# fverdoja/Fast-3D-Pointcloud-Segmentation

Measured on AMD Instinct MI355X. Metric: Mpoints/sec segmented end-to-end, 1M-pt RGB-D frames, higher is better.
Workload: dtype f32

## Files before the change

### __graft_entry__.py

```python
import importlib
import os
import subprocess
import sys

ROOT = os.path.dirname(os.path.abspath(__file__))
PKG = "fast-3d-pointcloud-segmentation_amd"


def _run(cmd):
    print("+", " ".join(cmd), flush=True)
    subprocess.run(cmd, check=True)


def build() -> None:
    _run(["make", "-C", os.path.join(ROOT, PKG, "csrc")])
    _run(["make", "-C", os.path.join(ROOT, "oracle")])
    _run(["make", "-C", os.path.join(ROOT, "tests", "emul")])
    _run(["make", "-C", os.path.join(ROOT, "tests", "devprobe")])
    _run(["make", "-C", os.path.join(ROOT, "tests", "kernprobe")])
    if ROOT not in sys.path:
        sys.path.insert(0, ROOT)
    P = importlib.import_module(PKG)
    lib = P.load_library()
    assert lib.f3ds_version() >= 120
    P.check_library_is_current(lib)


def smoke() -> None:
    import ctypes
    import numpy as np
    if ROOT not in sys.path:
        sys.path.insert(0, ROOT)
    sys.path.insert(0, os.path.join(ROOT, "tests"))
    P = importlib.import_module(PKG)
    from conftest import CpuChecker
    if P.device_count() < 1:
        raise RuntimeError("smoke(): no HIP device visible; libf3ds has no CPU fallback")
    pts = P.synth_frame(0, 7, 160, 120, 30)
    prm = P.launch_params(voxel_res=0.02, seed_res=0.2)
    ctx = P.Context(0)
    labels = ctx.segment(pts, prm)
    ora = CpuChecker(os.path.join(ROOT, "oracle", "libf3ds_oracle.so"), "f3ds_oracle")
    rc, olabels, ores, oh = ora.segment(pts, prm)
    assert rc == 0
    assert np.array_equal(labels, olabels), "HIP labels differ from the oracle"
    assert ctx.result.n_regions == ores.n_regions and ctx.result.n_merges == ores.n_merges
    print("smoke ok: N=%d V=%d S=%d E=%d merges=%d regions=%d  (%.2f ms on device 0)" % (
        len(pts), ctx.result.n_voxels, ctx.result.n_supervoxels, ctx.result.n_edges, ctx.result.n_merges, ctx.result.n_regions, ctx.result.ms_total))
    ctx.close()


if __name__ == "__main__":
# ... 4 lines not shown
```

### fast-3d-pointcloud-segmentation_amd/csrc/f3ds_hip.hip

```cpp
#include <hip/hip_runtime.h>

#include <algorithm>
#include <cmath>
#include <atomic>
#include <map>
#include <chrono>
#include <cstdio>
#include <cstdlib>
#include <cstring>
#include <string>
#include <type_traits>
#include <mutex>
#include <set>
#include <vector>

#include "../../include/f3ds.h"
#include "f3ds_algo.h"
#include "f3ds_glasbey.h"
#include "f3ds_eval.h"
#include "f3ds_dev.h"
#include "f3ds_levels.h"
#include "f3ds_eval_levels.h"

using namespace f3ds;
// ... 425 lines not shown
    rec<d_scan_single>(c, 1u, 0u, tiles, nt);
    rec<d_seg_write>(c, nt, 0u, c->ks, n, invalid, ks, tiles, seg_start, &c->d_dc->n_voxels, &c->d_dc->n_valid);
    return F3DS_OK;
}
int seg_vox_tiles(f3ds_ctx* c, int code_bits, int tile_bits) {
    const uint32_t n = c->n;
    const uint32_t ntiles = (n + VT_TILE - 1u) / VT_TILE;
    const uint64_t dcap64 = (uint64_t)ntiles * VT_ENT_MAX;
    if (code_bits + tile_bits + VT_CNT_BITS > 64 || dcap64 > 0x7fffffffull || (uint64_t)ntiles * VT_TAB > 0x7fffffffull) return F3DS_ERR_UNSUPPORTED;
    const uint32_t dcap = (uint32_t)dcap64;
    const uint64_t fin = c->h_dc->n_finite;
    const uint32_t capV = (uint32_t)std::max<uint64_t>(256u, std::min<uint64_t>(fin, dcap));
    c->vox_cap = capV;
    uint64_t *k0, *k1; uint32_t *ploc, *v0, *v1, *part, *vkey, *vcount, *seg_start, *list; uint2* bo_te; float* vf; int* pt_voxel;
    const uint32_t nchunks = (dcap + DS_CHUNK - 1u) / DS_CHUNK;
    ENSURE(c->pslot, n, ploc); ENSURE(c->keys0, dcap, k0); ENSURE(c->keys1, dcap, k1); ENSURE(c->vals0, dcap, v0); ENSURE(c->vals1, dcap, v1);
    { uint32_t* w; ENSURE(c->hcnt, (size_t)ntiles * VT_TAB * 2 + 2u * nchunks, w); bo_te = reinterpret_cast<uint2*>(w); part = w + (size_t)ntiles * VT_TAB * 2; }
    ENSURE(c->vkey, (size_t)capV * 3, vkey); ENSURE(c->vcount, capV, vcount); ENSURE(c->vf, (size_t)capV * 12, vf);
    ENSURE(c->seg_start, (size_t)capV + 1, seg_start); ENSURE(c->vlist, n, list); ENSURE(c->pt_voxel, n, pt_voxel);
    { uint32_t *f, *incl; ENSURE(c->flags, capV, f); ENSURE(c->incl, capV, incl); }
    c->idxbits = -1; c->ks = nullptr; c->vs = nullptr;
    rec<d_tile_keys>(c, std::min<uint32_t>(ntiles, (uint32_t)g_grid_cap * 16u), 0u, c->d_pts, n, c->fa, c->d_grid, ploc, k0, v0, dcap, tile_bits, c->d_dc);
    uint64_t* ks; uint32_t* vs;
    int rc = radix_sort(c, k0, v0, k1, v1, dcap, code_bits + tile_bits, &ks, &vs, VT_CNT_BITS, &c->d_dc->seg_count);
    if (rc) return rc;
    rec<d_desc_part>(c, nchunks, 0u, ks, dcap, tile_bits, part, c->d_dc);
    rec<d_desc_offsets>(c, 1u, 0u, part, dcap, capV, seg_start, c->d_dc);
    rec<d_desc_apply>(c, nchunks, 0u, ks, vs, dcap, capV, tile_bits, c->fa, c->d_grid, part, bo_te, seg_start, vkey, c->d_dc);
    rec<d_tile_place>(c, std::min<uint32_t>(ntiles, (uint32_t)g_grid_cap * 16u), 0u, ploc, n, bo_te, list, pt_voxel, c->d_dc);
    rec<d_voxel_list_accum>(c, std::min<uint32_t>(grid_wide(capV, 256), std::max<uint32_t>(64u, grid_wide(n / 8u, 256))), 0u, c->d_pts, list, seg_start, c->fa, vf, vcount, c->d_dc, capV);
    c->vox_hashed = true;
    return F3DS_OK;
}
int seg_voxels(f3ds_ctx* c) {
    const uint32_t V = c->V, n = c->n;
    uint32_t *vkey, *vcount, *hvals; float *vf; int *nbr, *nbrT; uint64_t* hkeys;
    if (c->vox_hashed) {
        const uint32_t hc2 = pow2_ge((size_t)V * 2 + 16);
        c->hmask = hc2 - 1;
        ENSURE(c->nbr, (size_t)V * 27, nbr); ENSURE(c->nbrT, (size_t)V * 27, nbrT); ENSURE(c->hkeys, hc2, hkeys); ENSURE(c->hvals, hc2, hvals);
        rec_fill(c, hkeys, 0xFFFFFFFFu, (size_t)hc2 * 8);
        rec<d_vox_hash>(c, 1u, 0u, c->vkey.p, V, c->d_grid, hkeys, hvals, c->hmask);
        rec<d_neighbors>(c, grid_wide((size_t)V * 27, 256), 0u, c->vkey.p, c->d_dc, c->d_grid, hkeys, hvals, c->hmask, nbr, nbrT);
        return F3DS_OK;
    }
    const uint32_t hcap = pow2_ge((size_t)V * 2 + 16);
    c->hmask = hcap - 1;
    ENSURE(c->vkey, (size_t)V * 3, vkey); ENSURE(c->vcount, V, vcount); ENSURE(c->vf, (size_t)V * 12, vf);
    ENSURE(c->nbr, (size_t)V * 27, nbr); ENSURE(c->nbrT, (size_t)V * 27, nbrT); ENSURE(c->hkeys, hcap, hkeys); ENSURE(c->hvals, hcap, hvals);
    rec_fill(c, hkeys, 0xFFFFFFFFu, (size_t)hcap * 8);
    if (g_sw.split_voxel_accum) {
        P16* spts; ENSURE(c->spts, n, spts);
        rec<d_point_gather>(c, grid_wide(n, 256), 0u, c->d_pts, c->vs, c->ks, c->idxbits < 0 ? 0 : c->idxbits, c->incl.p, n, c->d_dc, spts, c->pt_voxel.p);
        rec<d_voxel_accum>(c, grid_wide(V, 256), 0u, spts, c->ks, c->idxbits < 0 ? 0 : c->idxbits, c->seg_start.p, c->d_dc, c->fa, c->d_grid, vkey, vcount, vf, hkeys, hvals, c->hmask);
    } else
        rec<d_voxel_gather_accum>(c, grid_wide(V, 256), 0u, c->d_pts, c->vs, c->ks, c->idxbits < 0 ? 0 : c->idxbits, c->seg_start.p, n, c->d_dc, c->fa, c->d_grid, vkey, vcount, vf, hkeys, hvals, c->hmask, c->pt_voxel.p);
    rec<d_neighbors>(c, grid_wide((size_t)V * 27, 256), 0u, vkey, c->d_dc, c->d_grid, hkeys, hvals, c->hmask, nbr, nbrT);
    return F3DS_OK;
}
int seg_normals(f3ds_ctx* c) {
    const uint32_t nt = (c->V + NT_TILE - 1) / NT_TILE;
    uint32_t *tn1, *tord, *tslots;
    ENSURE(c->tile_n1, nt, tn1); ENSURE(c->tile_ord, (size_t)nt * NT_RING1, tord); ENSURE(c->tile_slots, (size_t)nt * SW_SLOT_WORDS * NT_TILE, tslots);
#ifdef F3DS_NORMALS_LOOP
    static const uint32_t budget = dev_getenv("F3DS_NORMALS_WGS") ? (uint32_t)atoi(dev_getenv("F3DS_NORMALS_WGS")) : 0u;
#else
    static const uint32_t budget = 0u;
#endif
    const uint32_t share = budget ? std::max(2u, budget / (uint32_t)g_batch_frames) : nt;
    const int nthr_env = g_sw.normals_threads;
    const uint32_t holes = g_sw.tile_holes;
    if (nthr_env ? nthr_env == 256 : g_batch_frames >= 16)
        rec<d_normals_t<256>>(c, std::min(nt, share), 0u, c->vf.p, c->nbr.p, c->d_dc, tn1, tord, tslots, holes);
    else
        rec<d_normals_t<384>>(c, std::min(nt, share), 0u, c->vf.p, c->nbr.p, c->d_dc, tn1, tord, tslots, holes);
    return F3DS_OK;
}
int seg_seed_grid(f3ds_ctx* c) {
    const uint32_t V = c->V;
    float* boxes; const float* vf = c->vf.p;
    const uint32_t nchunks = (V + SEED_CHUNK - 1) / SEED_CHUNK;
    ENSURE(c->boxes, (size_t)nchunks * 6, boxes);
    rec<d_chunkbox>(c, nchunks, 0u, vf, c->d_dc, boxes);
    rec<d_seed_grow>(c, 1u, 0u, vf, boxes, c->d_dc, c->prm.seed_res, c->d_sgrid);
    return F3DS_OK;
}
int seg_seed_cells(f3ds_ctx* c, int sort_bits, int max_sdepth) {
    const uint32_t V = c->V;
    uint32_t *ckey, *cell_start, *v0, *v1; uint64_t *k0 = c->keys0.p, *k1 = c->keys1.p;
    ENSURE(c->vals0, V, v0); ENSURE(c->vals1, V, v1);
    ENSURE(c->ckey, (size_t)V * 3, ckey); ENSURE(c->cell_start, (size_t)V + 1, cell_start);
// ... 1484 lines not shown
```

### fast-3d-pointcloud-segmentation_amd/csrc/f3ds_kernels.inc

```


namespace {

struct P16 { float x, y, z; uint32_t rgba; };

struct DevCounters {
    unsigned long long n_finite;
    uint32_t bbox[6];
    uint32_t bbox_any;
    uint32_t n_valid;
    uint32_t n_voxels;
    uint32_t n_cells;
    uint32_t n_seeds;
    uint32_t n_edges;
    uint32_t n_alive;
    uint32_t n_merges;
    uint32_t n_regions;
    uint32_t n_events;
    int error;
    int r_overflow;
    float lambda;
    uint32_t seg_count;
    uint32_t n_ghosts;
    int depth;
// ... 245 lines not shown
        __syncthreads();
    #pragma unroll
        for (int s = 0; s < RS_STRIPS; ++s) {
            uint32_t i = wbase + s * 64 + lane_id();
            const bool valid = i < n;
            const uint32_t d = (uint32_t)(k[s] >> shift) & mask;
            uint64_t peers = __ballot(valid);
            for (int b = 0; b < bits; ++b) {
                uint64_t m = __ballot(valid && ((d >> b) & 1u));
                peers &= ((d >> b) & 1u) ? m : ~m;
            }
            uint32_t pos = 0;
            if (valid) pos = wcount[w][d] + (uint32_t)__popcll(peers & lanemask_lt());
            __builtin_amdgcn_wave_barrier();
            if (valid && (peers & lanemask_lt()) == 0ull) wcount[w][d] += (uint32_t)__popcll(peers);
            __builtin_amdgcn_wave_barrier();
            if (valid) keys_out[pos] = k[s];
        }
    }
};

struct FrameArgs {
    int use_transform, fold_negative_z, leaf_order;
    float voxel_res, seed_res, w_color, w_spatial, w_normal;
};

__device__ inline P16 load_point(const P16* pts, size_t i) {
    const uint4 q = reinterpret_cast<const uint4*>(pts)[i];
    P16 p;
    p.x = __uint_as_float(q.x); p.y = __uint_as_float(q.y); p.z = __uint_as_float(q.z); p.rgba = q.w;
    return p;
}

__device__ inline bool vt_compact(int depth) { return depth <= 10; }
__device__ inline uint32_t vt_key30(unsigned x, unsigned y, unsigned z) { return (x << 20) | (y << 10) | z; }
template <bool WG_SCOPE>
__device__ inline void vt_insert(uint64_t* hkeys, uint32_t* hvals, uint32_t hmask, int depth, unsigned x, unsigned y, unsigned z, uint32_t v) {
    const bool compact = vt_compact(depth);
    const unsigned long long pk = compact ? (((unsigned long long)vt_key30(x, y, z) << 32) | v) : (unsigned long long)n_pack_key(x, y, z);
    uint32_t h = (uint32_t)hash64(compact ? (uint64_t)vt_key30(x, y, z) : (uint64_t)pk) & hmask;
    for (;;) {
        unsigned long long expect = HASH_EMPTY;
        const bool won = WG_SCOPE ? __hip_atomic_compare_exchange_strong((unsigned long long*)&hkeys[h], &expect, pk, __ATOMIC_RELAXED, __ATOMIC_RELAXED, __HIP_MEMORY_SCOPE_WORKGROUP)
                                  : __hip_atomic_compare_exchange_strong((unsigned long long*)&hkeys[h], &expect, pk, __ATOMIC_RELAXED, __ATOMIC_RELAXED, __HIP_MEMORY_SCOPE_AGENT);
        if (won || (!compact && expect == pk)) { if (!compact) hvals[h] = v; return; }
        h = (h + 1u) & hmask;
    }
}
__device__ inline int vt_find(const uint64_t* hkeys, const uint32_t* hvals, uint32_t hmask, bool compact, unsigned x, unsigned y, unsigned z) {
    if (compact) {
        const uint32_t ck = vt_key30(x, y, z);
        uint32_t h = (uint32_t)hash64((uint64_t)ck) & hmask;
        for (;;) {
            const uint64_t e = hkeys[h];
            if ((uint32_t)(e >> 32) == ck) return (int)(uint32_t)e;
            if (e == HASH_EMPTY) return -1;
            h = (h + 1u) & hmask;
        }
    }
    const uint64_t pk = n_pack_key(x, y, z);
    uint32_t h = (uint32_t)hash64(pk) & hmask;
    for (;;) {
        const uint64_t k = hkeys[h];
        if (k == pk) return (int)hvals[h];
        if (k == HASH_EMPTY) return -1;
        h = (h + 1u) & hmask;
    }
}
struct d_bbox {
    static constexpr int BLOCK = 256;
    __device__ void operator()(const P16* pts, uint32_t n, FrameArgs fa, DevCounters* dc) const {
        float mn[3] = {F3DS_FLT_MAX, F3DS_FLT_MAX, F3DS_FLT_MAX}, mx[3] = {-F3DS_FLT_MAX, -F3DS_FLT_MAX, -F3DS_FLT_MAX};
        uint32_t nfin = 0, any = 0;
        for (uint32_t i = BIX * blockDim.x + threadIdx.x; i < n; i += gridDim.x * blockDim.x) {
            P16 p = load_point(pts, i);
            float x = p.x, y = p.y, z = p.z;
            n_prelude(z, fa.fold_negative_z);
            if (n_finite3(x, y, z)) nfin++;
            n_transform(x, y, z, fa.use_transform);
            if (!n_finite3(x, y, z)) continue;
            any = 1;
            if (x < mn[0]) mn[0] = x;
            if (y < mn[1]) mn[1] = y;
            if (z < mn[2]) mn[2] = z;
            if (x > mx[0]) mx[0] = x;
            if (y > mx[1]) mx[1] = y;
            if (z > mx[2]) mx[2] = z;
        }
    #pragma unroll
        for (int d = 32; d >= 1; d >>= 1) {
            for (int a = 0; a < 3; ++a) {
                float t = __shfl_xor(mn[a], d, 64); if (t < mn[a]) mn[a] = t;
                t = __shfl_xor(mx[a], d, 64); if (t > mx[a]) mx[a] = t;
            }
            nfin += __shfl_xor(nfin, d, 64);
            any |= __shfl_xor(any, d, 64);
        }
        __shared__ float smn[4][3], smx[4][3];
        __shared__ uint32_t sfin[4], sany[4];
// ... 100 lines not shown
    __device__ void operator()(const uint64_t* keys, uint32_t n, uint64_t limit, int shift, const uint32_t* tile_offsets, uint32_t* seg_start, uint32_t* nseg_out, uint32_t* nvalid_out) const {
        if (BIX > 0 && BIX * SCAN_TILE >= n) return;
        const uint32_t base = BIX * SCAN_TILE + threadIdx.x * SCAN_ITEMS;
        uint64_t k[SCAN_ITEMS + 1]; uint32_t mask, tot;
        const uint32_t cnt = seg_heads_of_thread(keys, n, limit, shift, base, k, &mask);
        uint32_t run = tile_offsets[BIX] + block_incl_scan<SCAN_THREADS>(cnt, &tot) - cnt;
#pragma unroll
        for (int i = 0; i < SCAN_ITEMS; ++i) {
            const uint32_t pos = base + (uint32_t)i;
            if (mask & (1u << i)) seg_start[run++] = pos;
            if (pos < n && k[i] < limit && (pos + 1u == n || k[i + 1] >= limit)) { seg_start[run] = pos + 1u; *nseg_out = run; *nvalid_out = pos + 1u; }
        }
    }
};
struct d_point_gather {
    static constexpr int BLOCK = 256;
    __device__ void operator()(const P16* pts, const uint32_t* vals, const uint64_t* keys, int idxbits, const uint32_t* incl, uint32_t n, const DevCounters* dc, P16* spts,
                               int* pt_voxel) const {
        const uint32_t nv = dc->n_valid;
        for (uint32_t i = BIX * blockDim.x + threadIdx.x; i < n; i += gridDim.x * blockDim.x) {
            const uint32_t idx = vals ? vals[i] : (uint32_t)(keys[i] & ((1ull << idxbits) - 1ull));
            if (i < nv) {
                const P16 p = load_point(pts, idx);
                *reinterpret_cast<float4*>(spts + i) = make_float4(p.x, p.y, p.z, __uint_as_float(p.rgba));
                pt_voxel[idx] = (int)(incl[i] - 1u);
            } else pt_voxel[idx] = -1;
        }
    }
};
struct d_voxel_accum {
    static constexpr int BLOCK = 256;
    __device__ void operator()(const P16* spts, const uint64_t* keys, int keyshift, const uint32_t* seg_start,
                                                    const DevCounters* dc, FrameArgs fa, const GridInfo* gp, uint32_t* vkey, uint32_t* vcount,
                                                    float* vf, uint64_t* hkeys, uint32_t* hvals, uint32_t hmask) const {
        const uint32_t V = dc->n_voxels;
        const int depth = gp->depth;
        for (uint32_t v = BIX * blockDim.x + threadIdx.x; v < V; v += gridDim.x * blockDim.x) {
            const uint32_t s = seg_start[v], e = seg_start[v + 1];
            float sx = 0, sy = 0, sz = 0, sr = 0, sg = 0, sb = 0;
            for (uint32_t i = s; i < e; ++i) {
                P16 p = load_point(spts, i);
                float z = p.z; n_prelude(z, fa.fold_negative_z);
                sx += p.x; sy += p.y; sz += z;
                sr += (float)((p.rgba >> 16) & 255u); sg += (float)((p.rgba >> 8) & 255u); sb += (float)(p.rgba & 255u);
            }
            const uint32_t cnt = e - s;
            const float c = (float)cnt;
            float4* row = reinterpret_cast<float4*>(vf + (size_t)v * 12);
            row[0] = make_float4(sx / c, sy / c, sz / c, sr / c);
            row[1] = make_float4(sg / c, sb / c, 0.0f, 0.0f);
            row[2] = make_float4(0.0f, 0.0f, 0.0f, 0.0f);
            vcount[v] = cnt;
            uint64_t code = keys[s] >> keyshift;
            if (fa.leaf_order == 1) code = (~code) & ((1ull << (3 * depth)) - 1ull);
            unsigned k[3];
            n_demorton(code, depth, k);
            vkey[v * 3] = k[0]; vkey[v * 3 + 1] = k[1]; vkey[v * 3 + 2] = k[2];
            vt_insert<false>(hkeys, hvals, hmask, depth, k[0], k[1], k[2], v);
        }
    }
};
constexpr uint32_t VG_CHUNK = 1024;
struct d_voxel_gather_accum {
    static constexpr int BLOCK = 256;
    __device__ void operator()(const P16* pts, const uint32_t* vals, const uint64_t* keys, int keyshift, const uint32_t* seg_start, uint32_t n,
                               const DevCounters* dc, FrameArgs fa, const GridInfo* gp, uint32_t* vkey, uint32_t* vcount,
                               float* vf, uint64_t* hkeys, uint32_t* hvals, uint32_t hmask, int* pt_voxel) const {
        __shared__ __attribute__((aligned(16))) uint4 buf[VG_CHUNK];
        __shared__ uint32_t ibuf[VG_CHUNK], vbuf[VG_CHUNK];
        const uint32_t V = dc->n_voxels, nv = dc->n_valid;
        const int depth = gp->depth;
        const uint64_t imask = (1ull << keyshift) - 1ull;
        const uint32_t tid = threadIdx.x;
        for (uint32_t i = nv + BIX * blockDim.x + tid; i < n; i += gridDim.x * blockDim.x) pt_voxel[vals ? vals[i] : (uint32_t)(keys[i] & imask)] = -1;
        for (uint32_t vb = BIX * 256u; vb < V; vb += gridDim.x * 256u) {
            const uint32_t v = vb + tid;
            const bool mine = v < V;
            const uint32_t s = mine ? seg_start[v] : 0u, e = mine ? seg_start[v + 1] : 0u;
            const uint32_t p0 = seg_start[vb], p1 = seg_start[vb + 256u < V ? vb + 256u : V];
            float sx = 0, sy = 0, sz = 0, sr = 0, sg = 0, sb = 0;
            for (uint32_t c0 = p0; c0 < p1; c0 += VG_CHUNK) {
                const uint32_t c1 = p1 - c0 < VG_CHUNK ? p1 : c0 + VG_CHUNK;
                uint32_t idx[VG_CHUNK / 256];
        #pragma unroll
                for (uint32_t j = 0; j < VG_CHUNK / 256; ++j) { const uint32_t i = c0 + j * 256u + tid; const uint32_t ii = i < c1 ? i : c1 - 1u; idx[j] = vals ? vals[ii] : (uint32_t)(keys[ii] & imask); }
                uint4 q[VG_CHUNK / 256];
        #pragma unroll
                for (uint32_t j = 0; j < VG_CHUNK / 256; ++j) q[j] = reinterpret_cast<const uint4*>(pts)[idx[j]];
        #pragma unroll
                for (uint32_t j = 0; j < VG_CHUNK / 256; ++j) { buf[j * 256u + tid] = q[j]; ibuf[j * 256u + tid] = idx[j]; }
                __syncthreads();
                const uint32_t a = s > c0 ? s : c0, b = e < c1 ? e : c1;
                for (uint32_t i = a; i < b; ++i) {
                    const uint4 w = buf[i - c0];
                    float z = __uint_as_float(w.z); n_prelude(z, fa.fold_negative_z);
                    sx += __uint_as_float(w.x); sy += __uint_as_float(w.y); sz += z;
                    sr += (float)((w.w >> 16) & 255u); sg += (float)((w.w >> 8) & 255u); sb += (float)(w.w & 255u);
                    vbuf[i - c0] = v;
                }
                __syncthreads();
        #pragma unroll
                for (uint32_t j = 0; j < VG_CHUNK / 256; ++j) { const uint32_t pp = j * 256u + tid; if (c0 + pp < c1) pt_voxel[ibuf[pp]] = (int)vbuf[pp]; }
                __syncthreads();
            }
            if (!mine) continue;
            const uint32_t cnt = e - s;
            const float c = (float)cnt;
            float4* row = reinterpret_cast<float4*>(vf + (size_t)v * 12);
            row[0] = make_float4(sx / c, sy / c, sz / c, sr / c);
            row[1] = make_float4(sg / c, sb / c, 0.0f, 0.0f);
            row[2] = make_float4(0.0f, 0.0f, 0.0f, 0.0f);
            vcount[v] = cnt;
            uint64_t code = keys[s] >> keyshift;
            if (fa.leaf_order == 1) code = (~code) & ((1ull << (3 * depth)) - 1ull);
            unsigned k[3];
            n_demorton(code, depth, k);
            vkey[v * 3] = k[0]; vkey[v * 3 + 1] = k[1]; vkey[v * 3 + 2] = k[2];
            vt_insert<false>(hkeys, hvals, hmask, depth, k[0], k[1], k[2], v);
        }
    }
};

#ifndef F3DS_VT_TILE
#define F3DS_VT_TILE 4096
#endif
constexpr uint32_t VT_TILE = F3DS_VT_TILE;
constexpr uint32_t VT_TAB = VT_TILE / 2;
constexpr int VT_CNT_BITS = 14;
static_assert(VT_TILE < (1u << VT_CNT_BITS), "a tile's point count must fit the count field");
constexpr uint32_t VT_ENT_MAX = VT_TAB * 5 / 8;
constexpr uint32_t VL_MAX_RUN = 256;
constexpr uint32_t VOX_NONE = 0xFFFFFFFFu;
__device__ inline void run_of_lane(bool valid, uint32_t w0, uint32_t w1, bool* head, int* head_lane, uint32_t* run_len) {
    const int lane = lane_id();
    const uint32_t p0 = __shfl_up(w0, 1, 64), p1 = __shfl_up(w1, 1, 64);
    const bool pv = __shfl_up((int)valid, 1, 64) != 0;
    const bool h = valid && (lane == 0 || !pv || p0 != w0 || p1 != w1);
    const uint64_t hm = __ballot(h), vm = __ballot(valid);
    const uint64_t le = lane == 63 ? ~0ull : ((2ull << lane) - 1ull);
    const int hl = valid ? 63 - __builtin_clzll(hm & le) : lane;
    const uint64_t above = hl == 63 ? 0ull : ~((2ull << hl) - 1ull);
    const uint64_t stop = (hm | ~vm) & above;
    *head = h; *head_lane = hl; *run_len = (uint32_t)((stop ? __builtin_ctzll(stop) : 64) - hl);
}
struct d_tile_keys {
    static constexpr int BLOCK = 256;
    __device__ void operator()(const P16* pts, uint32_t n, FrameArgs fa, const GridInfo* gp, uint32_t* ploc, uint64_t* dkeys, uint32_t* dvals,
                               uint32_t dcap, int tile_bits, DevCounters* dc) const {
        __shared__ unsigned long long tkey[VT_TAB];
        __shared__ uint32_t tcnt[VT_TAB];
        __shared__ uint32_t tbits[2][VT_TAB / 32];
// ... 198 lines not shown
    static constexpr int BLOCK = 256;
    __device__ void operator()(const uint32_t* ploc, uint32_t n, const uint2* bo_te, uint32_t* list, int* pt_voxel, const DevCounters* dc) const {
        __shared__ uint2 tab[VT_TAB];
        if (dc->ev_overflow) return;
        const uint32_t ntiles = (n + VT_TILE - 1u) / VT_TILE;
        for (uint32_t tile = BIX; tile < ntiles; tile += gridDim.x) {
            const uint32_t t0 = tile * VT_TILE, t1 = n - t0 < VT_TILE ? n : t0 + VT_TILE;
            constexpr uint32_t PF = 4;
            uint32_t pl[PF];
    #pragma unroll
            for (uint32_t j = 0; j < PF; ++j) { const uint32_t i = t0 + j * 256u + threadIdx.x; pl[j] = i < t1 ? ploc[i] : VOX_NONE; }
            __syncthreads();
            for (uint32_t e = threadIdx.x; e < VT_TAB; e += 256u) tab[e] = bo_te[(size_t)tile * VT_TAB + e];
            __syncthreads();
            for (uint32_t i0 = t0; i0 < t1; i0 += 256u * PF) {
                uint32_t nx[PF];
    #pragma unroll
                for (uint32_t j = 0; j < PF; ++j) { const uint32_t i = i0 + (PF + j) * 256u + threadIdx.x; nx[j] = i < t1 ? ploc[i] : VOX_NONE; }
    #pragma unroll
                for (uint32_t j = 0; j < PF; ++j) {
                    const uint32_t i = i0 + j * 256u + threadIdx.x;
                    if (i >= t1) continue;
                    if (pl[j] == VOX_NONE) { pt_voxel[i] = -1; continue; }
                    const uint2 bo = tab[pl[j] >> 16];
                    list[bo.x + (pl[j] & 0xFFFFu)] = i;
                    pt_voxel[i] = (int)bo.y;
                }
    #pragma unroll
                for (uint32_t j = 0; j < PF; ++j) pl[j] = nx[j];
            }
        }
    }
};
struct d_vox_hash {
    static constexpr bool LATENCY_KERNEL = true;
    static constexpr int BLOCK = 1024;
    __device__ void operator()(const uint32_t* vkey, uint32_t V, const GridInfo* gp, uint64_t* hkeys, uint32_t* hvals, uint32_t hmask) const {
        if (BIX) return;
        const int depth = gp->depth;
        constexpr uint32_t PF = 4;
        for (uint32_t v0 = threadIdx.x; v0 < V; v0 += blockDim.x * PF) {
            unsigned k[PF][3];
    #pragma unroll
            for (uint32_t j = 0; j < PF; ++j) { const uint32_t v = v0 + j * blockDim.x, vv = v < V ? v : 0u; k[j][0] = vkey[vv * 3]; k[j][1] = vkey[vv * 3 + 1]; k[j][2] = vkey[vv * 3 + 2]; }
    #pragma unroll
            for (uint32_t j = 0; j < PF; ++j) { const uint32_t v = v0 + j * blockDim.x; if (v < V) vt_insert<true>(hkeys, hvals, hmask, depth, k[j][0], k[j][1], k[j][2], v); }
        }
    }
};
struct d_voxel_list_accum {
    static constexpr int BLOCK = 256;
    __device__ void operator()(const P16* pts, uint32_t* list, const uint32_t* seg_start, FrameArgs fa, float* vf, uint32_t* vcount, DevCounters* dc, uint32_t capV) const {
        __shared__ __attribute__((aligned(16))) uint4 buf[VG_CHUNK];
        if (dc->ev_overflow) return;
        const uint32_t V = dc->n_voxels < capV ? dc->n_voxels : capV;
        const bool disorder = dc->vox_disorder != 0u;
        const uint32_t tid = threadIdx.x;
        for (uint32_t vb = BIX * 256u; vb < V; vb += gridDim.x * 256u) {
            const uint32_t v = vb + tid;
            const bool mine = v < V;
            const uint32_t s = mine ? seg_start[v] : 0u, e = mine ? seg_start[v + 1] : 0u;
            const uint32_t p0 = seg_start[vb], p1 = seg_start[vb + 256u < V ? vb + 256u : V];
            if (__syncthreads_or(e - s > VL_MAX_RUN)) { if (tid == 0) { dc->error = F3DS_ERR_UNSUPPORTED; dc->ev_overflow = 6; } return; }
            if (disorder) {
                for (uint32_t a = s + 1u; a < e; ++a) {
                    const uint32_t x = list[a];
                    uint32_t b = a;
                    while (b > s && list[b - 1u] > x) { list[b] = list[b - 1u]; --b; }
                    if (b != a) list[b] = x;
                }
                __threadfence_block();
                __syncthreads();
            }
            float sx = 0, sy = 0, sz = 0, sr = 0, sg = 0, sb = 0;
            for (uint32_t c0 = p0; c0 < p1; c0 += VG_CHUNK) {
                const uint32_t c1 = p1 - c0 < VG_CHUNK ? p1 : c0 + VG_CHUNK;
                uint32_t idx[VG_CHUNK / 256];
        #pragma unroll
                for (uint32_t j = 0; j < VG_CHUNK / 256; ++j) { const uint32_t i = c0 + j * 256u + tid; idx[j] = list[i < c1 ? i : c1 - 1u]; }
// ... 4 lines not shown
                for (uint32_t j = 0; j < VG_CHUNK / 256; ++j) buf[j * 256u + tid] = q[j];
                __syncthreads();
                const uint32_t a = s > c0 ? s : c0, b = e < c1 ? e : c1;
                for (uint32_t i = a; i < b; ++i) {
                    const uint4 w = buf[i - c0];
                    float z = __uint_as_float(w.z); n_prelude(z, fa.fold_negative_z);
                    sx += __uint_as_float(w.x); sy += __uint_as_float(w.y); sz += z;
                    sr += (float)((w.w >> 16) & 255u); sg += (float)((w.w >> 8) & 255u); sb += (float)(w.w & 255u);
                }
                __syncthreads();
            }
            if (!mine) continue;
            const float c = (float)(e - s);
            vcount[v] = e - s;
            float4* row = reinterpret_cast<float4*>(vf + (size_t)v * 12);
            row[0] = make_float4(sx / c, sy / c, sz / c, sr / c);
            row[1] = make_float4(sg / c, sb / c, 0.0f, 0.0f);
            row[2] = make_float4(0.0f, 0.0f, 0.0f, 0.0f);
        }
    }
};
__device__ inline int hash_find(const uint64_t* hkeys, const uint32_t* hvals, uint32_t hmask, uint64_t pk) {
    uint32_t h = (uint32_t)hash64(pk) & hmask;
    for (;;) {
        uint64_t k = hkeys[h];
        if (k == pk) return (int)hvals[h];
        if (k == HASH_EMPTY) return -1;
        h = (h + 1u) & hmask;
    }
}

struct d_neighbors {
    static constexpr int BLOCK = 256;
    __device__ void operator()(const uint32_t* vkey, const DevCounters* dc, const GridInfo* gp, const uint64_t* hkeys,
                                                  const uint32_t* hvals, uint32_t hmask, int* nbr, int* nbrT) const {
        __shared__ int tr[27][65];
        const uint32_t V = dc->n_voxels;
        const unsigned max_key = gp->max_key;
        const bool compact = vt_compact(gp->depth);
        for (uint32_t vb = BIX * 64u; vb < V; vb += gridDim.x * 64u) {
            const uint32_t nv = V - vb < 64u ? V - vb : 64u, np = nv * 27u;
            for (uint32_t tl = threadIdx.x; tl < np; tl += 256u) {
                const uint32_t vl = tl / 27u, s = tl - vl * 27u, v = vb + vl;
                const int d[3] = {(int)(s / 9u) - 1, (int)((s / 3u) % 3u) - 1, (int)(s % 3u) - 1};
                bool ok = true; unsigned k[3];
                for (int a = 0; a < 3; ++a) {
                    long long q = (long long)vkey[v * 3 + a] + d[a];
                    if (q < 0 || q > (long long)max_key) ok = false;
                    k[a] = (unsigned)q;
                }
                const int u = ok ? vt_find(hkeys, hvals, hmask, compact, k[0], k[1], k[2]) : -1;
                nbr[(size_t)vb * 27u + tl] = u;
                tr[s][vl] = u;
            }
            __syncthreads();
            for (uint32_t r = threadIdx.x; r < 27u * 64u; r += 256u) {
                const uint32_t s = r >> 6, vl = r & 63u;
                if (vl < nv) nbrT[(size_t)s * V + vb + vl] = tr[s][vl];
            }
            __syncthreads();
        }
    }
};
constexpr int NT_TILE = 128;
constexpr int NT_HCAP = 2048;
#ifndef F3DS_NT_SLOTS
#define F3DS_NT_SLOTS 896
#endif
#ifndef F3DS_NT_RING1
#define F3DS_NT_RING1 448
#endif
constexpr int NT_SLOTS = F3DS_NT_SLOTS;
constexpr int NT_RING1 = F3DS_NT_RING1;
constexpr uint16_t NT_NONE = 0xFFFFu;
constexpr uint32_t NT_HNONE = 0x3FFu;
constexpr uint32_t NT_ORD_LIMIT = (1u << 22) - 2u;
static_assert(NT_SLOTS < 1023, "slot numbers share a word with the ordinal");
constexpr uint16_t NT_ZERO = NT_SLOTS;
constexpr uint32_t SW_TILE_NONE = 0xFFFFFFFFu;
constexpr int SW_SLOT_BITS = 9;
constexpr int SW_SLOT_WORDS = (27 * SW_SLOT_BITS + 31) / 32;
static_assert(NT_RING1 < (1 << SW_SLOT_BITS), "a list position must fit its bit field");
__device__ __forceinline__ void sw_slots_pack(const uint32_t pos[27], uint32_t w[SW_SLOT_WORDS]) {
#pragma unroll
// ... 3034 lines not shown
```

### fast-3d-pointcloud-segmentation_amd/csrc/f3ds_numerics.h

```cpp
#ifndef F3DS_NUMERICS_H_
#define F3DS_NUMERICS_H_

#include "f3ds_math.h"

namespace f3ds {

#define F3DS_FLT_MAX 3.402823466e+38f
#define F3DS_FLT_MIN 1.175494351e-38f
#define F3DS_FLT_EPS 1.192092896e-07f

F3DS_HD float n_sqrtf(float x) { return __builtin_sqrtf(x); }
F3DS_HD double n_sqrt(double x) { return __builtin_sqrt(x); }
F3DS_HD bool n_finite3(float x, float y, float z) { return m_isfinitef(x) && m_isfinitef(y) && m_isfinitef(z); }
F3DS_HD float n_nanf() { return m_from_bitsf(0x7fc00000u); }

struct GridInfo {
    double min[3];
    double max[3];
    double res;
    int depth;
    unsigned max_key;
    int error;
    int empty;
};
// ... 55 lines not shown
    v = (v | (v << 8)) & 0x0300F00Fu;
    v = (v | (v << 4)) & 0x030C30C3u;
    v = (v | (v << 2)) & 0x09249249u;
    return v;
}
F3DS_HD uint64_t n_spread3_21(uint64_t v) {
    v = (v | (v << 32)) & 0x001F00000000FFFFull;
    v = (v | (v << 16)) & 0x001F0000FF0000FFull;
    v = (v | (v << 8)) & 0x100F00F00F00F00Full;
    v = (v | (v << 4)) & 0x10C30C30C30C30C3ull;
    v = (v | (v << 2)) & 0x1249249249249249ull;
    return v;
}
F3DS_HD uint64_t n_morton(unsigned x, unsigned y, unsigned z, int depth) {
    if (depth <= 10) {
        const uint32_t m = (1u << depth) - 1u;
        return (uint64_t)((n_spread3_10(x & m) << 2) | (n_spread3_10(y & m) << 1) | n_spread3_10(z & m));
    }
    const uint64_t m = (1ull << depth) - 1ull;
    return (n_spread3_21(x & m) << 2) | (n_spread3_21(y & m) << 1) | n_spread3_21(z & m);
}
F3DS_HD void n_demorton(uint64_t c, int depth, unsigned key[3]) {
    unsigned x = 0, y = 0, z = 0;
    for (int b = depth - 1; b >= 0; --b) {
        unsigned d = (unsigned)(c >> (3 * b)) & 7u;
        x = (x << 1) | ((d >> 2) & 1u);
        y = (y << 1) | ((d >> 1) & 1u);
        z = (z << 1) | (d & 1u);
    }
    key[0] = x; key[1] = y; key[2] = z;
}
F3DS_HD uint64_t n_pack_key(unsigned x, unsigned y, unsigned z) {
    return ((uint64_t)x << 42) | ((uint64_t)y << 21) | (uint64_t)z;
}

F3DS_HD void n_roots2(float b, float c, float r[3]) {
    r[0] = 0.0f;
    float d = (float)((double)(b * b) - 4.0 * (double)c);
    if (d < 0.0f) d = 0.0f;
    float sd = n_sqrtf(d);
    r[2] = 0.5f * (b + sd);
    r[1] = 0.5f * (b - sd);
}
template <class K = m_lit> F3DS_HD void n_roots(float m00, float m01, float m02, float m11, float m12, float m22, float r[3], K mc = K()) {
    float c0 = m00 * m11 * m22 + 2.0f * m01 * m02 * m12 - m00 * m12 * m12 - m11 * m02 * m02 - m22 * m01 * m01;
    float c1 = m00 * m11 - m01 * m01 + m00 * m22 - m02 * m02 + m11 * m22 - m12 * m12;
    float c2 = m00 + m11 + m22;
    if (m_absf(c0) < F3DS_FLT_EPS) { n_roots2(c2, c1, r); return; }
    const float inv3 = (float)(1.0 / 3.0);
    const float sqrt3 = 1.7320508075688772f;
    float c2_3 = c2 * inv3;
    float a_3 = (c1 - c2 * c2_3) * inv3;
    if (a_3 > 0.0f) a_3 = 0.0f;
    float half_b = 0.5f * (c0 + c2_3 * (2.0f * c2_3 * c2_3 - c1));
    float q = half_b * half_b + a_3 * a_3 * a_3;
    if (q > 0.0f) q = 0.0f;
    float rho = n_sqrtf(-a_3);
    float theta = m_atan2f(n_sqrtf(-q), half_b, mc) * inv3;
    float ct = m_cosf(theta, mc), st = m_sinf(theta, mc);
    r[0] = c2_3 + 2.0f * rho * ct;
    r[1] = c2_3 - rho * (ct + sqrt3 * st);
    r[2] = c2_3 - rho * (ct - sqrt3 * st);
    float t;
    if (r[0] >= r[1]) { t = r[0]; r[0] = r[1]; r[1] = t; }
    if (r[1] >= r[2]) {
        t = r[1]; r[1] = r[2]; r[2] = t;
// ... 188 lines not shown
```

Baseline: 3638.

## Replace per-voxel hash table with 4x4x4 block occupancy table for neighbor lookup

```diff
diff --git a/__graft_entry__.py b/__graft_entry__.py
--- a/__graft_entry__.py
+++ b/__graft_entry__.py
@@ -18,6 +18,7 @@
     _run(["make", "-C", os.path.join(ROOT, "tests", "emul")])
     _run(["make", "-C", os.path.join(ROOT, "tests", "devprobe")])
     _run(["make", "-C", os.path.join(ROOT, "tests", "kernprobe")])
+    _run(["make", "-C", os.path.join(ROOT, "tests", "blockprobe")])
     if ROOT not in sys.path:
         sys.path.insert(0, ROOT)
     P = importlib.import_module(PKG)
diff --git a/fast-3d-pointcloud-segmentation_amd/csrc/f3ds_hip.hip b/fast-3d-pointcloud-segmentation_amd/csrc/f3ds_hip.hip
--- a/fast-3d-pointcloud-segmentation_amd/csrc/f3ds_hip.hip
+++ b/fast-3d-pointcloud-segmentation_amd/csrc/f3ds_hip.hip
@@ -481,31 +481,32 @@
     c->vox_hashed = true;
     return F3DS_OK;
 }
+int seg_neighbors(f3ds_ctx* c, uint32_t wgs) {
+    const uint32_t V = c->V;
+    const bool blocks = c->h_dc->depth <= N_BLOCK_DEPTH_MAX;
+    const uint32_t cap = blocks ? pow2_ge((size_t)V + 16) : pow2_ge((size_t)V * 2 + 16);
+    const size_t words = blocks ? (size_t)cap * 2 : cap;
+    uint32_t* hvals = nullptr; int *nbr, *nbrT; uint64_t* hkeys;
+    c->hmask = cap - 1;
+    ENSURE(c->nbr, (size_t)V * 27, nbr); ENSURE(c->nbrT, (size_t)V * 27, nbrT); ENSURE(c->hkeys, words, hkeys);
+    if (!blocks) ENSURE(c->hvals, cap, hvals);
+    rec_fill(c, hkeys, 0xFFFFFFFFu, words * 8);
+    rec<d_vox_table>(c, wgs, 0u, c->vkey.p, V, c->d_grid, hkeys, hvals, c->hmask);
+    rec<d_neighbors>(c, grid_wide((size_t)V * 27, 256), 0u, c->vkey.p, c->d_dc, c->d_grid, c->fa.leaf_order, hkeys, hvals, c->hmask, nbr, nbrT);
+    return F3DS_OK;
+}
 int seg_voxels(f3ds_ctx* c) {
     const uint32_t V = c->V, n = c->n;
-    uint32_t *vkey, *vcount, *hvals; float *vf; int *nbr, *nbrT; uint64_t* hkeys;
-    if (c->vox_hashed) {
-        const uint32_t hc2 = pow2_ge((size_t)V * 2 + 16);
-        c->hmask = hc2 - 1;
-        ENSURE(c->nbr, (size_t)V * 27, nbr); ENSURE(c->nbrT, (size_t)V * 27, nbrT); ENSURE(c->hkeys, hc2, hkeys); ENSURE(c->hvals, hc2, hvals);
-        rec_fill(c, hkeys, 0xFFFFFFFFu, (size_t)hc2 * 8);
-        rec<d_vox_hash>(c, 1u, 0u, c->vkey.p, V, c->d_grid, hkeys, hvals, c->hmask);
-        rec<d_neighbors>(c, grid_wide((size_t)V * 27, 256), 0u, c->vkey.p, c->d_dc, c->d_grid, hkeys, hvals, c->hmask, nbr, nbrT);
-        return F3DS_OK;
-    }
-    const uint32_t hcap = pow2_ge((size_t)V * 2 + 16);
-    c->hmask = hcap - 1;
+    if (c->vox_hashed) return seg_neighbors(c, 1u);
+    uint32_t *vkey, *vcount; float *vf;
     ENSURE(c->vkey, (size_t)V * 3, vkey); ENSURE(c->vcount, V, vcount); ENSURE(c->vf, (size_t)V * 12, vf);
-    ENSURE(c->nbr, (size_t)V * 27, nbr); ENSURE(c->nbrT, (size_t)V * 27, nbrT); ENSURE(c->hkeys, hcap, hkeys); ENSURE(c->hvals, hcap, hvals);
-    rec_fill(c, hkeys, 0xFFFFFFFFu, (size_t)hcap * 8);
     if (g_sw.split_voxel_accum) {
         P16* spts; ENSURE(c->spts, n, spts);
         rec<d_point_gather>(c, grid_wide(n, 256), 0u, c->d_pts, c->vs, c->ks, c->idxbits < 0 ? 0 : c->idxbits, c->incl.p, n, c->d_dc, spts, c->pt_voxel.p);
-        rec<d_voxel_accum>(c, grid_wide(V, 256), 0u, spts, c->ks, c->idxbits < 0 ? 0 : c->idxbits, c->seg_start.p, c->d_dc, c->fa, c->d_grid, vkey, vcount, vf, hkeys, hvals, c->hmask);
+        rec<d_voxel_accum>(c, grid_wide(V, 256), 0u, spts, c->ks, c->idxbits < 0 ? 0 : c->idxbits, c->seg_start.p, c->d_dc, c->fa, c->d_grid, vkey, vcount, vf);
     } else
-        rec<d_voxel_gather_accum>(c, grid_wide(V, 256), 0u, c->d_pts, c->vs, c->ks, c->idxbits < 0 ? 0 : c->idxbits, c->seg_start.p, n, c->d_dc, c->fa, c->d_grid, vkey, vcount, vf, hkeys, hvals, c->hmask, c->pt_voxel.p);
-    rec<d_neighbors>(c, grid_wide((size_t)V * 27, 256), 0u, vkey, c->d_dc, c->d_grid, hkeys, hvals, c->hmask, nbr, nbrT);
-    return F3DS_OK;
+        rec<d_voxel_gather_accum>(c, grid_wide(V, 256), 0u, c->d_pts, c->vs, c->ks, c->idxbits < 0 ? 0 : c->idxbits, c->seg_start.p, n, c->d_dc, c->fa, c->d_grid, vkey, vcount, vf, c->pt_voxel.p);
+    return seg_neighbors(c, grid_for(V, 4096));
 }
 int seg_normals(f3ds_ctx* c) {
     const uint32_t nt = (c->V + NT_TILE - 1) / NT_TILE;
diff --git a/fast-3d-pointcloud-segmentation_amd/csrc/f3ds_kernels.inc b/fast-3d-pointcloud-segmentation_amd/csrc/f3ds_kernels.inc
--- a/fast-3d-pointcloud-segmentation_amd/csrc/f3ds_kernels.inc
+++ b/fast-3d-pointcloud-segmentation_amd/csrc/f3ds_kernels.inc
@@ -301,32 +301,24 @@
     return p;
 }
 
-__device__ inline bool vt_compact(int depth) { return depth <= 10; }
-__device__ inline uint32_t vt_key30(unsigned x, unsigned y, unsigned z) { return (x << 20) | (y << 10) | z; }
-template <bool WG_SCOPE>
-__device__ inline void vt_insert(uint64_t* hkeys, uint32_t* hvals, uint32_t hmask, int depth, unsigned x, unsigned y, unsigned z, uint32_t v) {
-    const bool compact = vt_compact(depth);
-    const unsigned long long pk = compact ? (((unsigned long long)vt_key30(x, y, z) << 32) | v) : (unsigned long long)n_pack_key(x, y, z);
-    uint32_t h = (uint32_t)hash64(compact ? (uint64_t)vt_key30(x, y, z) : (uint64_t)pk) & hmask;
+__device__ inline bool vt_blocks(int depth) { return depth <= N_BLOCK_DEPTH_MAX; }
+constexpr uint32_t BT_EMPTY = 0xFFFFFFFFu;
+struct __attribute__((aligned(16))) BtEntry { uint32_t key, base; unsigned long long vacant; };
+static_assert(sizeof(BtEntry) == 16, "one 16-byte load per probe");
+template <class T> __device__ inline bool vt_cas(T* p, T* expect, T v, bool agent) {
+    return agent ? __hip_atomic_compare_exchange_strong(p, expect, v, __ATOMIC_RELAXED, __ATOMIC_RELAXED, __HIP_MEMORY_SCOPE_AGENT)
+                 : __hip_atomic_compare_exchange_strong(p, expect, v, __ATOMIC_RELAXED, __ATOMIC_RELAXED, __HIP_MEMORY_SCOPE_WORKGROUP);
+}
+__device__ inline void vt_insert(uint64_t* hkeys, uint32_t* hvals, uint32_t hmask, bool agent, unsigned x, unsigned y, unsigned z, uint32_t v) {
+    const unsigned long long pk = (unsigned long long)n_pack_key(x, y, z);
+    uint32_t h = (uint32_t)hash64((uint64_t)pk) & hmask;
     for (;;) {
         unsigned long long expect = HASH_EMPTY;
-        const bool won = WG_SCOPE ? __hip_atomic_compare_exchange_strong((unsigned long long*)&hkeys[h], &expect, pk, __ATOMIC_RELAXED, __ATOMIC_RELAXED, __HIP_MEMORY_SCOPE_WORKGROUP)
-                                  : __hip_atomic_compare_exchange_strong((unsigned long long*)&hkeys[h], &expect, pk, __ATOMIC_RELAXED, __ATOMIC_RELAXED, __HIP_MEMORY_SCOPE_AGENT);
-        if (won || (!compact && expect == pk)) { if (!compact) hvals[h] = v; return; }
+        if (vt_cas((unsigned long long*)&hkeys[h], &expect, pk, agent) || expect == pk) { hvals[h] = v; return; }
         h = (h + 1u) & hmask;
     }
 }
-__device__ inline int vt_find(const uint64_t* hkeys, const uint32_t* hvals, uint32_t hmask, bool compact, unsigned x, unsigned y, unsigned z) {
-    if (compact) {
-        const uint32_t ck = vt_key30(x, y, z);
-        uint32_t h = (uint32_t)hash64((uint64_t)ck) & hmask;
-        for (;;) {
-            const uint64_t e = hkeys[h];
-            if ((uint32_t)(e >> 32) == ck) return (int)(uint32_t)e;
-            if (e == HASH_EMPTY) return -1;
-            h = (h + 1u) & hmask;
-        }
-    }
+__device__ inline int vt_find(const uint64_t* hkeys, const uint32_t* hvals, uint32_t hmask, unsigned x, unsigned y, unsigned z) {
     const uint64_t pk = n_pack_key(x, y, z);
     uint32_t h = (uint32_t)hash64(pk) & hmask;
     for (;;) {
@@ -334,6 +326,24 @@
         if (k == pk) return (int)hvals[h];
         if (k == HASH_EMPTY) return -1;
         h = (h + 1u) & hmask;
+    }
+}
+__device__ inline BtEntry* bt_entry(BtEntry* tab, uint32_t tmask, bool agent, uint32_t bk) {
+    uint32_t h = (uint32_t)hash64((uint64_t)bk) & tmask;
+    for (;;) {
+        uint32_t expect = BT_EMPTY;
+        if (vt_cas(&tab[h].key, &expect, bk, agent) || expect == bk) return &tab[h];
+        h = (h + 1u) & tmask;
+    }
+}
+__device__ inline int bt_find(const BtEntry* tab, uint32_t tmask, int leaf_order, unsigned x, unsigned y, unsigned z) {
+    const uint32_t bk = n_block_key(x, y, z);
+    uint32_t h = (uint32_t)hash64((uint64_t)bk) & tmask;
+    for (;;) {
+        const uint4 e = reinterpret_cast<const uint4*>(tab)[h];
+        if (e.x == bk) return n_block_ordinal(e.y, ~(((uint64_t)e.w << 32) | (uint64_t)e.z), n_block_cell(x, y, z), leaf_order);
+        if (e.x == BT_EMPTY) return -1;
+        h = (h + 1u) & tmask;
     }
 }
 struct d_bbox {
@@ -500,7 +510,7 @@
     static constexpr int BLOCK = 256;
     __device__ void operator()(const P16* spts, const uint64_t* keys, int keyshift, const uint32_t* seg_start,
                                                     const DevCounters* dc, FrameArgs fa, const GridInfo* gp, uint32_t* vkey, uint32_t* vcount,
-                                                    float* vf, uint64_t* hkeys, uint32_t* hvals, uint32_t hmask) const {
+                                                    float* vf) const {
         const uint32_t V = dc->n_voxels;
         const int depth = gp->depth;
         for (uint32_t v = BIX * blockDim.x + threadIdx.x; v < V; v += gridDim.x * blockDim.x) {
@@ -524,7 +534,6 @@
             unsigned k[3];
             n_demorton(code, depth, k);
             vkey[v * 3] = k[0]; vkey[v * 3 + 1] = k[1]; vkey[v * 3 + 2] = k[2];
-            vt_insert<false>(hkeys, hvals, hmask, depth, k[0], k[1], k[2], v);
         }
     }
 };
@@ -533,7 +542,7 @@
     static constexpr int BLOCK = 256;
     __device__ void operator()(const P16* pts, const uint32_t* vals, const uint64_t* keys, int keyshift, const uint32_t* seg_start, uint32_t n,
                                const DevCounters* dc, FrameArgs fa, const GridInfo* gp, uint32_t* vkey, uint32_t* vcount,
-                               float* vf, uint64_t* hkeys, uint32_t* hvals, uint32_t hmask, int* pt_voxel) const {
+                               float* vf, int* pt_voxel) const {
         __shared__ __attribute__((aligned(16))) uint4 buf[VG_CHUNK];
         __shared__ uint32_t ibuf[VG_CHUNK], vbuf[VG_CHUNK];
         const uint32_t V = dc->n_voxels, nv = dc->n_valid;
@@ -584,7 +593,6 @@
             unsigned k[3];
             n_demorton(code, depth, k);
             vkey[v * 3] = k[0]; vkey[v * 3 + 1] = k[1]; vkey[v * 3 + 2] = k[2];
-            vt_insert<false>(hkeys, hvals, hmask, depth, k[0], k[1], k[2], v);
         }
     }
 };
@@ -849,19 +857,51 @@
         }
     }
 };
-struct d_vox_hash {
+struct d_vox_table {
     static constexpr bool LATENCY_KERNEL = true;
     static constexpr int BLOCK = 1024;
     __device__ void operator()(const uint32_t* vkey, uint32_t V, const GridInfo* gp, uint64_t* hkeys, uint32_t* hvals, uint32_t hmask) const {
-        if (BIX) return;
-        const int depth = gp->depth;
+        const bool blocks = vt_blocks(gp->depth);
+        const bool agent = gridDim.x > 1u;
+        BtEntry* const tab = reinterpret_cast<BtEntry*>(hkeys);
+        const uint32_t lane = (uint32_t)lane_id();
         constexpr uint32_t PF = 4;
-        for (uint32_t v0 = threadIdx.x; v0 < V; v0 += blockDim.x * PF) {
-            unsigned k[PF][3];
-    #pragma unroll
-            for (uint32_t j = 0; j < PF; ++j) { const uint32_t v = v0 + j * blockDim.x, vv = v < V ? v : 0u; k[j][0] = vkey[vv * 3]; k[j][1] = vkey[vv * 3 + 1]; k[j][2] = vkey[vv * 3 + 2]; }
-    #pragma unroll
-            for (uint32_t j = 0; j < PF; ++j) { const uint32_t v = v0 + j * blockDim.x; if (v < V) vt_insert<true>(hkeys, hvals, hmask, depth, k[j][0], k[j][1], k[j][2], v); }
+        for (uint32_t s0 = BIX * (BLOCK * PF); s0 < V; s0 += gridDim.x * (BLOCK * PF)) {
+            unsigned k[PF][3]; uint32_t prev[PF];
+    #pragma unroll
+            for (uint32_t j = 0; j < PF; ++j) { const uint32_t v = s0 + j * BLOCK + threadIdx.x, vv = v < V ? v : 0u; k[j][0] = vkey[vv * 3]; k[j][1] = vkey[vv * 3 + 1]; k[j][2] = vkey[vv * 3 + 2]; }
+            if (!blocks) {
+    #pragma unroll
+                for (uint32_t j = 0; j < PF; ++j) { const uint32_t v = s0 + j * BLOCK + threadIdx.x; if (v < V) vt_insert(hkeys, hvals, hmask, agent, k[j][0], k[j][1], k[j][2], v); }
+                continue;
+            }
+    #pragma unroll
+            for (uint32_t j = 0; j < PF; ++j) {
+                const uint32_t v = s0 + j * BLOCK + threadIdx.x;
+                prev[j] = lane == 0u && v > 0u && v < V ? n_block_key(vkey[(v - 1u) * 3], vkey[(v - 1u) * 3 + 1], vkey[(v - 1u) * 3 + 2]) : BT_EMPTY;
+            }
+    #pragma unroll
+            for (uint32_t j = 0; j < PF; ++j) {
+                const uint32_t v = s0 + j * BLOCK + threadIdx.x;
+                const bool in = v < V;
+                const uint32_t bk = n_block_key(k[j][0], k[j][1], k[j][2]);
+                const uint32_t up = __shfl_up(bk, 1, 64);
+                const bool head = in && bk != (lane ? up : prev[j]);
+                const uint64_t cuts = __ballot(head || !in);
+                const uint64_t ahead = (cuts >> 1) >> lane;
+                unsigned long long m = in ? 1ull << n_block_cell(k[j][0], k[j][1], k[j][2]) : 0ull;
+    #pragma unroll
+                for (uint32_t d = 1; d < 64u; d <<= 1) {
+                    const unsigned long long o = __shfl_down(m, d, 64);
+                    if (lane + d < 64u && !(ahead & ((1ull << d) - 1ull))) m |= o;
+                }
+                if (in && (head || lane == 0u)) {
+                    BtEntry* const e = bt_entry(tab, hmask, agent, bk);
+                    if (agent) __hip_atomic_fetch_and(&e->vacant, ~m, __ATOMIC_RELAXED, __HIP_MEMORY_SCOPE_AGENT);
+                    else __hip_atomic_fetch_and(&e->vacant, ~m, __ATOMIC_RELAXED, __HIP_MEMORY_SCOPE_WORKGROUP);
+                    if (head) e->base = v;
+                }
+            }
         }
     }
 };
@@ -932,12 +972,13 @@
 
 struct d_neighbors {
     static constexpr int BLOCK = 256;
-    __device__ void operator()(const uint32_t* vkey, const DevCounters* dc, const GridInfo* gp, const uint64_t* hkeys,
+    __device__ void operator()(const uint32_t* vkey, const DevCounters* dc, const GridInfo* gp, int leaf_order, const uint64_t* hkeys,
                                                   const uint32_t* hvals, uint32_t hmask, int* nbr, int* nbrT) const {
         __shared__ int tr[27][65];
         const uint32_t V = dc->n_voxels;
         const unsigned max_key = gp->max_key;
-        const bool compact = vt_compact(gp->depth);
+        const bool blocks = vt_blocks(gp->depth);
+        const BtEntry* const tab = reinterpret_cast<const BtEntry*>(hkeys);
         for (uint32_t vb = BIX * 64u; vb < V; vb += gridDim.x * 64u) {
             const uint32_t nv = V - vb < 64u ? V - vb : 64u, np = nv * 27u;
             for (uint32_t tl = threadIdx.x; tl < np; tl += 256u) {
@@ -949,7 +990,7 @@
                     if (q < 0 || q > (long long)max_key) ok = false;
                     k[a] = (unsigned)q;
                 }
-                const int u = ok ? vt_find(hkeys, hvals, hmask, compact, k[0], k[1], k[2]) : -1;
+                const int u = !ok ? -1 : blocks ? bt_find(tab, hmask, leaf_order, k[0], k[1], k[2]) : vt_find(hkeys, hvals, hmask, k[0], k[1], k[2]);
                 nbr[(size_t)vb * 27u + tl] = u;
                 tr[s][vl] = u;
             }
diff --git a/fast-3d-pointcloud-segmentation_amd/csrc/f3ds_numerics.h b/fast-3d-pointcloud-segmentation_amd/csrc/f3ds_numerics.h
--- a/fast-3d-pointcloud-segmentation_amd/csrc/f3ds_numerics.h
+++ b/fast-3d-pointcloud-segmentation_amd/csrc/f3ds_numerics.h
@@ -111,6 +111,14 @@
 }
 F3DS_HD uint64_t n_pack_key(unsigned x, unsigned y, unsigned z) {
     return ((uint64_t)x << 42) | ((uint64_t)y << 21) | (uint64_t)z;
+}
+#define N_BLOCK_DEPTH_MAX 12
+F3DS_HD uint32_t n_block_key(unsigned x, unsigned y, unsigned z) { return ((x >> 2) << 20) | ((y >> 2) << 10) | (z >> 2); }
+F3DS_HD unsigned n_block_cell(unsigned x, unsigned y, unsigned z) { return (unsigned)n_morton(x & 3u, y & 3u, z & 3u, 2); }
+F3DS_HD int n_block_ordinal(uint32_t base, uint64_t mask, unsigned cell, int leaf_order) {
+    if (!((mask >> cell) & 1ull)) return -1;
+    const uint64_t before = leaf_order == 1 ? ((mask >> cell) >> 1) : (mask & ((1ull << cell) - 1ull));
+    return (int)(base + (uint32_t)__builtin_popcountll(before));
 }
 
 F3DS_HD void n_roots2(float b, float c, float r[3]) {
```

Result: faster. 3730 (median of 6 runs) (+2.5%).
